# johanna-rock/quantization_analysis

Hardware: AMD Instinct MI355X
Metric: 32x32 tiles/s for mixed-tile-greedy (bf16->BFP{8,4,2}); achieved HBM GB/s vs peak (higher is better)
Workload: dtype f32/f64

## Files before the change

### include/mtq.h

```cpp
#ifndef MTQ_H
#define MTQ_H

#include <stddef.h>
#include <stdint.h>

#ifdef __cplusplus
extern "C" {
#endif

#define MTQ_VERSION 143

typedef enum {
    MTQ_OK = 0,
    MTQ_ERR_INVALID = -1,
    MTQ_ERR_HIP = -2,
    MTQ_ERR_NO_DEVICE = -3,
    MTQ_ERR_UNSUPPORTED = -4
} mtq_status;

enum { MTQ_DTYPE_BF16 = 0, MTQ_DTYPE_F32 = 1 };

enum { MTQ_FMT_BF16 = 0, MTQ_FMT_BFP8 = 1, MTQ_FMT_BFP4 = 2, MTQ_FMT_BFP2 = 3, MTQ_FMT_FP0 = 4, MTQ_FMT_MXFP4 = 5, MTQ_FMT_NVFP4 = 6 };
#define MTQ_NUM_TILE_FORMATS 4
#define MTQ_MASK_ALL 0xFu
// ... 130 lines not shown

int mtq_tile_scores_device(const double *stats, int64_t tiles, uint32_t fmt_mask, int metric, double *scores, void *stream);

int mtq_threshold_assign_device(const double *stats, int64_t tiles, uint32_t fmt_mask, const int *formats, int n_formats,
                                int metric, double threshold, double band, int8_t *map, uint8_t *knife, void *stream);


size_t mtq_columns_scratch_doubles(void);
int mtq_column_sums_device(const double *stats, int64_t tiles, uint32_t fmt_mask, const int8_t *map, double *scratch, void *stream);
int mtq_column_sums_device_batched(const double *stats, int64_t count, int64_t tiles, uint32_t fmt_mask, const int8_t *maps,
                                   double *scratch, void *stream);

#define MTQ_SCAN_DEVICE_MAX_TILES (1 << 22)
size_t mtq_greedy_scan_scratch_bytes(int64_t count, int64_t tiles);
int mtq_greedy_scan_device(const double *stats, int64_t count, int64_t tiles, uint32_t fmt_mask, const int *formats, int n_formats,
                           int metric, double threshold, double elem_count, const uint64_t *seeds, int8_t *maps, int32_t *status,
                           int32_t *counts, void *scratch, size_t scratch_bytes, void *stream);

size_t mtq_scan_carry_bytes(int64_t count);
int mtq_greedy_scan_device_ex(const double *stats, int64_t count, int64_t tiles, uint32_t fmt_mask, const int *formats, int n_formats,
                              int metric, double threshold, double elem_count, const uint64_t *seeds, int8_t *maps, int32_t *status,
                              int32_t *counts, void *scratch, size_t scratch_bytes, const void *orders, int phase, uint32_t *listed,
                              uint32_t *n_listed, void *carry, void *stream);
size_t mtq_scan_orders_bytes(int64_t tiles);
int mtq_scan_orders_device(uint64_t seed, int64_t tiles, int n_orders, void *orders, size_t orders_bytes, void *stream);

int mtq_knife_tiles_device(const void *x, int in_dtype, int64_t count, int64_t stride_elems, int64_t rows, int64_t cols, int64_t ld,
                           const int8_t *near, const int *formats, int n_formats, int64_t cap, int64_t *list, float *tiles_out, void *stream);

int mtq_knife_tiles_transposed(const void *x, int in_dtype, int64_t count, int64_t stride_elems, int64_t rows, int64_t cols, int64_t ld,
                               const int8_t *near, const int *formats, int n_formats, int64_t cap, int64_t *list, float *tiles_out, void *stream);

int mtq_threshold_enqueue(const void *x, int in_dtype, int64_t count, int64_t stride_elems, int64_t rows, int64_t cols, int64_t ld,
                          uint32_t k1_mask, uint32_t dec_mask, const int *formats, int n_formats, int metric, double threshold, double band,
                          double *stats, int8_t *both_dev, int8_t *both_host, int64_t cap, int64_t *list_dev, float *knife_dev,
                          int64_t *list_host, double *scratch, double *sums_host, void *stream, void *side_stream);
int mtq_threshold_enqueue_transposed(const void *x, int in_dtype, int64_t count, int64_t stride_elems, int64_t rows, int64_t cols, int64_t ld,
                                     uint32_t k1_mask, uint32_t dec_mask, const int *formats, int n_formats, int metric, double threshold, double band,
                                     double *stats, int8_t *both_dev, int8_t *both_host, int64_t cap, int64_t *list_dev, float *knife_dev,
                                     int64_t *list_host, double *scratch, double *sums_host, void *stream, void *side_stream);
int mtq_threshold_columns(const double *stats, int64_t count, int64_t tiles, uint32_t dec_mask, const int8_t *maps_dev, double *scratch,
                          double *sums_host, void *stream);

#define MTQ_RAGGED_MAX 24
typedef struct MtqMatrix { const void *x; int64_t rows, cols, ld; } MtqMatrix;
int mtq_tile_stats_ragged(const MtqMatrix *mats, int n, int in_dtype, uint32_t fmt_mask, double *stats, void *stream);
// ... 25 lines not shown
```

### quantization_analysis_amd/csrc/mtq_decide.hip

```cpp
#include <hip/hip_runtime.h>
#include <stdint.h>

#include "../../include/mtq.h"
#include "mtq_decide.hpp"
#include "mtq_error.hpp"

namespace mtq {

struct SlotTable { int slot[MTQ_NUM_TILE_FORMATS]; };

__global__ __launch_bounds__(256) void tile_scores_dev(const double *__restrict__ stats, int64_t tiles, int rec, SlotTable st, int metric,
                                                       double *__restrict__ scores)
{
    const int64_t t = (int64_t)blockIdx.x * 256 + threadIdx.x;
    if (t >= tiles) return;
    const double *r = stats + t * rec;
    int64_t row = 0;
#pragma unroll
    for (int f = 0; f < MTQ_NUM_TILE_FORMATS; ++f) {
        if (!slot_ok(st.slot[f])) continue;
        scores[row * tiles + t] = tile_score(r, st.slot[f], metric);
        ++row;
    }
}

__global__ __launch_bounds__(256) void threshold_assign_dev(const double *__restrict__ stats, int64_t tiles, int rec, ThresholdPlan plan,
                                                            int metric, double thr32, double band, int8_t *__restrict__ map,
                                                            uint8_t *__restrict__ knife)
{
    const int64_t t = (int64_t)blockIdx.x * 256 + threadIdx.x;
    if (t >= tiles) return;
    unsigned near;
    map[t] = (int8_t)threshold_decide(stats + t * rec, plan, metric, thr32, band, near);
    knife[t] = (uint8_t)near;
}

constexpr int kColBlocks = 256, kColVals = 11, kColMax = 6;

constexpr int kColSegs = 24;
struct ColSegs { uint32_t n; uint32_t first[kColSegs + 1]; };

__global__ __launch_bounds__(256) void columns_partial_dev(const double *__restrict__ stats, int64_t tiles, int rec, SlotTable st,
                                                           const int8_t *__restrict__ map, double *__restrict__ partial, int64_t scratch_stride,
                                                           const ColSegs seg)
{
    __shared__ double red[kColVals][256];
    int64_t stride_blocks = gridDim.x;
    if (seg.n) {
        const int64_t first = seg.first[blockIdx.y];
        tiles = (int64_t)seg.first[blockIdx.y + 1] - first;
        stride_blocks = (tiles + 255) / 256 < kColBlocks ? (tiles + 255) / 256 : kColBlocks;
        if ((int64_t)blockIdx.x >= stride_blocks) return;
        stats += first * rec;
        map += first;
    } else {
        stats += (int64_t)blockIdx.y * tiles * rec;
        map += (int64_t)blockIdx.y * tiles;
    }
    partial += (int64_t)blockIdx.y * scratch_stride;
    double v[kColVals] = {0, 0, 0, 0, 0, 0, 0, 0, 0, 0, 0};
// ... 233 lines not shown
```

### quantization_analysis_amd/csrc/mtq_decide.hpp

```cpp
#pragma once
#include <stdint.h>

#include "../../include/mtq.h"

#if defined(__HIP__)
#define MTQ_HD __host__ __device__
#else
#define MTQ_HD
#endif

namespace mtq {

MTQ_HD inline int popcount4(uint32_t m) { return __builtin_popcount(m & MTQ_MASK_ALL); }

constexpr int kVirtualSlot = -2;

MTQ_HD inline int slot_of(uint32_t mask, int f)
{
    if (f < 0 || f >= MTQ_NUM_TILE_FORMATS) return -1;
    if (f == 0 && (mask & MTQ_MASK_BF16_IDENTITY) && !(mask & 1u)) return kVirtualSlot;
    if (!(mask & (1u << f))) return -1;
    return __builtin_popcount(mask & ((1u << f) - 1u));
}
MTQ_HD inline bool slot_ok(int slot) { return slot >= 0 || slot == kVirtualSlot; }

struct Sums5 { double y, y2, xy, ab, mx; };
MTQ_HD inline Sums5 load5(const double *r, int slot)
{
    if (slot >= 0) { const double *b = r + 2 + 5 * slot; return {b[0], b[1], b[2], b[3], b[4]}; }
    const double z = __builtin_fabs(r[0]) * 0.0;
    return {r[0], r[1], r[1], z, z};
}

MTQ_HD inline double nanmax(double m, double d) { return (d > m || d != d) ? d : m; }

MTQ_HD inline bool is_good(double v, int metric, double thr) { return metric == MTQ_METRIC_PCC ? v >= thr : v <= thr; }

MTQ_HD inline double pcc_from_moments(double n, double sx, double sx2, double sy, double sy2, double sxy, double sab)
{
    if (n == 0.0) return 1.0;
    const double mean_x = sx / n;
    const double mean_y = sy / n;
    double am2 = sx2 - n * mean_x * mean_x;
    double bm2 = sy2 - n * mean_y * mean_y;
    if (am2 < 0.0) am2 = 0.0;
    if (bm2 < 0.0) bm2 = 0.0;
    const double denom = __builtin_sqrt(am2 * bm2);
    if (denom == 0.0) return sab == 0.0 ? 1.0 : 0.0;
    return (sxy - n * mean_x * mean_y) / denom;
}

MTQ_HD inline double tile_score(const double *r, int slot, int metric)
{
    const Sums5 b = load5(r, slot);
    if (metric == MTQ_METRIC_MAE) return b.ab / 1024.0;
    if (metric == MTQ_METRIC_ATOL) return b.mx;
    return pcc_from_moments(1024.0, r[0], r[1], b.y, b.y2, b.xy, b.ab);
// ... 52 lines not shown
```

### quantization_analysis_amd/csrc/mtq_scan.hip

```cpp
#include <hip/hip_runtime.h>
#include <stdint.h>

#include <atomic>
#include <type_traits>
#include <stdlib.h>
#include <mutex>

#include "../../include/mtq.h"
#include "mtq_decide.hpp"
#include "mtq_error.hpp"

namespace mtq {
namespace {

constexpr int kScanMaxTilesLds = 32768;
constexpr int kTagSlots = 16384;
constexpr int kJump = 34;

} }
__device__ unsigned long long g_scan_ticks[16];
namespace mtq { namespace {

struct U128 { uint64_t lo, hi; };
__host__ __device__ inline U128 mul128(U128 a, U128 b)
// ... 232 lines not shown
struct ScanArgs {
    const double *stats;
    int64_t tiles;
    int rec;
    int n_formats;
    int fmt[MTQ_NUM_TILE_FORMATS];
    int oy[MTQ_NUM_TILE_FORMATS], oy2[MTQ_NUM_TILE_FORMATS], oxy[MTQ_NUM_TILE_FORMATS];
    int oab[MTQ_NUM_TILE_FORMATS];
    int omx[MTQ_NUM_TILE_FORMATS];
    int metric;
    double thr, n;
    const uint64_t *seeds;
    int8_t *maps;
    int32_t *status;
    int32_t *counts;
    uint32_t *order_g;
    double *delta;
    double *delta2;
    const U128 *jump_a, *jump_g;
    const unsigned char *orders;
    int phase;
    uint32_t *listed, *n_listed;
    Carry *carry;
};

constexpr int kNoOffset = 0xFF;
__device__ inline double rec_at(const double *rt, uint32_t off) { return off == (uint32_t)kNoOffset ? 0.0 : rt[off]; }

template <int kN>
__device__ inline void prefix_chain(const double *lds_d, double *lds_p, int lane, double s)
{
    double v[16], w[16];
#pragma unroll
    for (int u = 0; u < 16; ++u) v[u] = lds_d[u * 4 + lane];
#pragma unroll
    for (int i0 = 0; i0 < kN; i0 += 16) {
        if (i0 + 16 < kN) {
#pragma unroll
            for (int u = 0; u < 16; ++u) w[u] = lds_d[(i0 + 16 + u) * 4 + lane];
        }
#pragma unroll
        for (int u = 0; u < 16; ++u) { s = s + v[u]; lds_p[(i0 + u) * 4 + lane] = s; }
#pragma unroll
        for (int u = 0; u < 16; ++u) v[u] = w[u];
    }
}
// ... 25 lines not shown
    special = denom == 0.0;
    const double val = (sxy - n * mean_x * mean_y) / denom;
    return val >= thr;
}

#ifdef MTQ_SCAN_PROFILE
#define MTQ_SCAN_STAMP(slot) do { const unsigned long long now_ = clock64(); if (b == 0 && lane == 0 && (slot) < 16) g_scan_ticks[slot] = now_ - tick_s; tick_s = now_; } while (0)
#else
#define MTQ_SCAN_STAMP(slot) do { } while (0)
#endif

template <typename F>
__device__ __forceinline__ void sift_map(const int8_t *map, int T, int lane, F &&f)
{
    for (int t00 = 0; t00 < T; t00 += 64 * 8) {
        uint8_t b[8];
#pragma unroll
        for (int u = 0; u < 8; ++u) b[u] = (uint8_t)ld_l2(map + min(t00 + 64 * u + lane, T - 1));
#pragma unroll
        for (int u = 0; u < 8; ++u) b[u] = t00 + 64 * u + lane < T ? b[u] : (uint8_t)0x80u;
#pragma unroll
        for (int u = 0; u < 8; ++u)
            if (t00 + 64 * u < T) f(t00 + 64 * u, b[u]);
    }
}

struct Offsets3 { uint32_t y, y2, xy; };

template <bool kMae, typename TileAt, typename PrevOf>
__device__ inline void gather_deltas(const double *st, int rec, Offsets3 po, int f, int nc, double *delta, int lane, TileAt tile_at, PrevOf prev_of)
{
    const uint32_t oy_f = (po.y >> (8 * f)) & 0xFFu, oy2_f = (po.y2 >> (8 * f)) & 0xFFu, oxy_f = (po.xy >> (8 * f)) & 0xFFu;
    uint32_t nt[4];
#pragma unroll
    for (int u = 0; u < 4; ++u) {
        const int k = 64 * u + lane;
        nt[u] = k < nc ? tile_at((uint32_t)k) : 0u;
    }
    for (int k0 = 0; k0 < nc; k0 += 256) {
        uint32_t tt[4];
        int pv[4];
#pragma unroll
        for (int u = 0; u < 4; ++u) tt[u] = nt[u];
#pragma unroll
        for (int u = 0; u < 4; ++u) {
            const int k = k0 + 256 + 64 * u + lane;
// ... 418 lines not shown
        }
        if (lane == 0) {
            Carry &c = a.carry[b];
            c.Sy = Sy; c.Sy2 = Sy2; c.Sxy = Sxy; c.sum_x = sum_x; c.sum_x2 = sum_x2;
            c.state = r.state; c.inc = inc; c.has32 = r.has32 ? 1u : 0u; c.u32 = r.u32;
            c.status = status; c.done = (done || nc == 0) ? 1 : 0;
        }
        return;
    }

    int per_fmt[MTQ_NUM_TILE_FORMATS] = {0, 0, 0, 0};
    sift_map(map, T, lane, [&](int t0, uint8_t raw) {
        const int t = t0 + lane;
        int code = -1;
        if (t < T) { code = (int)(raw & 0x7Fu); map[t] = (int8_t)code; }
#pragma unroll
        for (int c = 0; c < MTQ_NUM_TILE_FORMATS; ++c) per_fmt[c] += __builtin_popcountll(__ballot(code == c));
    });
    if (lane == 0) {
        a.status[b] = status;
        if (a.counts)
            for (int c = 0; c < MTQ_NUM_TILE_FORMATS; ++c) a.counts[b * MTQ_NUM_TILE_FORMATS + c] = per_fmt[c];
    }
}

__global__ __launch_bounds__(256) void greedy_atol(ScanArgs a)
{
    __shared__ int s_bad, s_nan, s_cnt[MTQ_NUM_TILE_FORMATS];
    const int b = blockIdx.x;
    const int64_t T = a.tiles;
    const double *st = a.stats + (int64_t)b * T * a.rec;
    int8_t *map = a.maps + (int64_t)b * T;
    if (threadIdx.x == 0) { s_bad = 0; s_nan = 0; }
    if (threadIdx.x < MTQ_NUM_TILE_FORMATS) s_cnt[threadIdx.x] = 0;
    __syncthreads();
    const int base = a.fmt[0];
    bool bad = false, nan = false;
    for (int64_t t = threadIdx.x; t < T; t += 256) {
        const double *rt = st + t * a.rec;
        bad |= !(rec_at(rt, (uint32_t)a.omx[base]) <= a.thr);
        for (int p = 0; p < a.n_formats; ++p) { const double v = rec_at(rt, (uint32_t)a.omx[a.fmt[p]]); nan |= v != v; }
    }
    if (bad) s_bad = 1;
    if (nan) s_nan = 1;
    __syncthreads();
    const bool all_base = s_bad != 0;
// ... 177 lines not shown
{
    if (!orders) return fail(MTQ_ERR_INVALID, "null argument");
    if (seed == 0) return fail(MTQ_ERR_INVALID, "seed 0 means 'draw a random seed' in the reference; pass a non-zero seed");
    if (tiles <= 0 || tiles > MTQ_SCAN_DEVICE_MAX_TILES) return fail(MTQ_ERR_INVALID, "tiles out of range");
    if (n_orders < 1 || n_orders > 2) return fail(MTQ_ERR_INVALID, "n_orders must be 1 or 2");
    if (orders_bytes < mtq_scan_orders_bytes(tiles)) return fail(MTQ_ERR_INVALID, "orders is smaller than mtq_scan_orders_bytes()");
    if (int rc = require_device()) return rc;
    int dev = 0;
    if (hipGetDevice(&dev) != hipSuccess) return fail(MTQ_ERR_HIP, "hipGetDevice failed");
    const U128 *jt = jump_tables(dev);
    if (!jt) return fail(MTQ_ERR_HIP, "could not upload the jump-ahead tables");
    OrdersArgs a{seed, tiles, n_orders, static_cast<unsigned char *>(orders), jt, jt + kJump};
    hipStream_t st = static_cast<hipStream_t>(stream);
    if (hipMemsetAsync(orders, 0, sizeof(OrdersHdr), st) != hipSuccess) return fail(MTQ_ERR_HIP, "hipMemsetAsync failed");
    size_t lds = kTagSlots;
    if (tiles <= kScanMaxTilesLds) {
        lds += 2 * (size_t)((tiles + 7) & ~(int64_t)7);
        if (int rc = raise_lds(dev, 1, reinterpret_cast<const void *>(scan_orders), 2 * kScanMaxTilesLds + kTagSlots)) return rc;
    }
    hipLaunchKernelGGL(scan_orders, dim3((unsigned)n_orders), dim3(64), lds, st, a);
    return check_launch("mtq_scan_orders_device");
}

extern "C" int mtq_greedy_scan_device_ex(const double *stats, int64_t count, int64_t tiles, uint32_t fmt_mask, const int *formats, int n_formats,
                                         int metric, double threshold, double elem_count, const uint64_t *seeds, int8_t *maps, int32_t *status,
                                         int32_t *counts, void *scratch, size_t scratch_bytes, const void *orders, int phase, uint32_t *listed,
                                         uint32_t *n_listed, void *carry, void *stream)
{
    if (!stats || !formats || !seeds || !maps || !status || !scratch) return fail(MTQ_ERR_INVALID, "null argument");
    if (count <= 0 || count > (1 << 20) || tiles <= 0) return fail(MTQ_ERR_INVALID, "count and tiles must be positive");
    if (tiles > MTQ_SCAN_DEVICE_MAX_TILES) return fail(MTQ_ERR_UNSUPPORTED, "more tiles than the device scan takes: use the host scan");
    if (metric != MTQ_METRIC_PCC && metric != MTQ_METRIC_MAE && metric != MTQ_METRIC_ATOL) return fail(MTQ_ERR_INVALID, "unknown metric");
    if (n_formats <= 0 || n_formats > MTQ_NUM_TILE_FORMATS) return fail(MTQ_ERR_INVALID, "n_formats must be 1..4");
    if (fmt_mask & MTQ_MASK_SLIM) return fail(MTQ_ERR_INVALID, "the device scan reads full records");
    if (!(elem_count > 0.0)) return fail(MTQ_ERR_INVALID, "elem_count must be positive");
    if (scratch_bytes < mtq_greedy_scan_scratch_bytes(count, tiles)) return fail(MTQ_ERR_INVALID, "scratch is smaller than mtq_greedy_scan_scratch_bytes()");
    if (phase < 0 || phase > 2) return fail(MTQ_ERR_INVALID, "phase must be 0, 1 or 2");
    if (phase != 0) {
        if (metric == MTQ_METRIC_ATOL) return fail(MTQ_ERR_UNSUPPORTED, "the atol walk has no phases");
        if (n_formats < 2) return fail(MTQ_ERR_INVALID, "a split search needs at least two formats");
        if (!carry || (phase == 1 && (!listed || !n_listed))) return fail(MTQ_ERR_INVALID, "a split search needs carry (and listed, n_listed in phase 1)");
        if (count * tiles >= ((int64_t)1 << 32)) return fail(MTQ_ERR_INVALID, "too many tiles for the list of a split search");
    }
    ScanArgs a{};
    a.stats = stats;
    a.tiles = tiles;
    a.rec = 2 + 5 * popcount4(fmt_mask);
    a.n_formats = n_formats;
    for (int f = 0; f < MTQ_NUM_TILE_FORMATS; ++f) {
        const int s = slot_of(fmt_mask, f);
        a.oy[f] = s >= 0 ? 2 + 5 * s : 0;
        a.oy2[f] = s >= 0 ? 3 + 5 * s : 1;
        a.oxy[f] = s >= 0 ? 4 + 5 * s : 1;
        a.oab[f] = s >= 0 ? 5 + 5 * s : kNoOffset;
        a.omx[f] = s >= 0 ? 6 + 5 * s : kNoOffset;
    }
    a.metric = metric;
    for (int i = 0; i < n_formats; ++i) {
        if (!slot_ok(slot_of(fmt_mask, formats[i]))) return fail(MTQ_ERR_INVALID, "a format is not available under fmt_mask");
        for (int j = 0; j < i; ++j) if (formats[j] == formats[i]) return fail(MTQ_ERR_UNSUPPORTED, "the device scan needs distinct formats: use the host scan");
        a.fmt[i] = formats[i];
    }
    a.thr = threshold;
    a.n = elem_count;
    a.seeds = seeds;
    a.maps = maps;
    a.status = status;
    a.counts = counts;
    a.orders = static_cast<const unsigned char *>(orders);
    a.phase = phase;
    a.listed = listed;
    a.n_listed = n_listed;
    a.carry = static_cast<Carry *>(carry);
    if (int rc = require_device()) return rc;
    int dev = 0;
    if (hipGetDevice(&dev) != hipSuccess) return fail(MTQ_ERR_HIP, "hipGetDevice failed");
    const U128 *jt = jump_tables(dev);
    if (!jt) return fail(MTQ_ERR_HIP, "could not upload the jump-ahead tables");
    a.jump_a = jt;
    a.jump_g = jt + kJump;
    a.delta = static_cast<double *>(scratch);
    a.delta2 = a.delta + (size_t)count * (size_t)tiles * 4;
    a.order_g = reinterpret_cast<uint32_t *>(static_cast<unsigned char *>(scratch) + (size_t)count * (size_t)tiles * 8 * sizeof(double));
    hipStream_t st = static_cast<hipStream_t>(stream);
    if (metric == MTQ_METRIC_ATOL) {
        hipLaunchKernelGGL(greedy_atol, dim3((unsigned)count), dim3(256), 0, st, a);
        return check_launch("mtq_greedy_scan_device");
    }
    const unsigned threads = (orders && phase != 2) ? 128u : 64u;
    static int shared_lds = -1;
    if (shared_lds < 0) { const char *e = getenv("MTQ_SCAN_SHARED_LDS"); shared_lds = e ? atoi(e) : 0; }
    if (tiles <= kScanMaxTilesLds && !(threads == 128u && !shared_lds)) {
        const size_t lds = 2 * (size_t)((tiles + 7) & ~(int64_t)7) + kFixedLds;
        if (int rc = raise_lds(dev, 0, reinterpret_cast<const void *>(greedy_scan_pcc_lds), 2 * kScanMaxTilesLds + (int)kFixedLds)) return rc;
        hipLaunchKernelGGL(greedy_scan_pcc_lds, dim3((unsigned)count), dim3(threads), lds, st, a);
    } else {
        hipLaunchKernelGGL(greedy_scan_pcc_global, dim3((unsigned)count), dim3(threads), kFixedLds, st, a);
    }
    return check_launch("mtq_greedy_scan_device");
}

extern "C" int mtq_greedy_scan_device(const double *stats, int64_t count, int64_t tiles, uint32_t fmt_mask, const int *formats, int n_formats,
                                      int metric, double threshold, double elem_count, const uint64_t *seeds, int8_t *maps, int32_t *status,
                                      int32_t *counts, void *scratch, size_t scratch_bytes, void *stream)
{
    return mtq_greedy_scan_device_ex(stats, count, tiles, fmt_mask, formats, n_formats, metric, threshold, elem_count, seeds, maps, status, counts,
                                     scratch, scratch_bytes, nullptr, 0, nullptr, nullptr, nullptr, stream);
}
```

### quantization_analysis_amd/hip_backend.py

```python
from __future__ import annotations

import ctypes
import functools
import os
from pathlib import Path

import numpy as np

_PKG = Path(__file__).resolve().parent
LIB_PATH = Path(os.environ["MTQ_LIB"]).resolve() if os.environ.get("MTQ_LIB") else _PKG / "libmtq_hip.so"

MIXED_TILE_FORMATS = ["bf16", "bfp8", "bfp4", "bfp2"]
FMT_CODE = {"bf16": 0, "bfp8": 1, "bfp4": 2, "bfp2": 3, "fp0": 4}
PROXY_FORMATS = ["mxfp4", "nvfp4"]
QUANTIZE_CODE = {**FMT_CODE, "mxfp4": 5, "nvfp4": 6}
METRIC_CODE = {"pcc": 0, "mae": 1, "atol": 2}
DTYPE_BF16, DTYPE_F32 = 0, 1
TILE = 32

MTQ_VERSION = 143

SIGNATURES = {
    "mtq_version": ("i", "", False),
    "mtq_last_error": ("s", "", False),
# ... 18 lines not shown
    "mtq_greedy_value": ("i", "pp", False),
    "mtq_greedy_destroy": ("v", "p", False),
    "mtq_tile_scores": ("i", "pluip", False),
    "mtq_threshold_assign": ("i", "plupiiddppplp", False),
    "mtq_columns_from_stats": ("i", "plupdp", False),
    "mtq_columns_from_sums": ("i", "pdp", False),
    "mtq_tile_scores_device": ("i", "pluipp", False),
    "mtq_threshold_assign_device": ("i", "plupiiddppp", False),
    "mtq_columns_scratch_doubles": ("z", "", False),
    "mtq_column_sums_device": ("i", "pluppp", False),
    "mtq_column_sums_device_batched": ("i", "plluppp", False),
    "mtq_rng_create": ("i", "pq", False),
    "mtq_rng_permutation": ("i", "plp", False),
    "mtq_rng_integers": ("i", "pllp", False),
    "mtq_rng_destroy": ("v", "p", False),
    "mtq_greedy_run": ("i", "plupiiddqppp", False),
    "mtq_greedy_run_batch": ("i", "pllupiiddppppi", False),
    "mtq_selftest_slot_ring": ("i", "", False),
    "mtq_device_copy_2d": ("i", "pzpzzzp", False),
    "mtq_knife_tiles_device": ("i", "pilllllppilppp", False),
    "mtq_greedy_scan_scratch_bytes": ("z", "ll", False),
    "mtq_greedy_scan_device": ("i", "pllupiiddpppppzp", False),
    "mtq_greedy_scan_device_ex": ("i", "pllupiiddpppppzpipppp", False),
    "mtq_scan_carry_bytes": ("z", "l", False),
    "mtq_scan_orders_bytes": ("z", "l", False),
    "mtq_scan_orders_device": ("i", "qlipzp", False),
    "mtq_debug_scan_ticks": ("i", "p", False),
    "mtq_threshold_enqueue": ("i", "pillllluupiiddppplppppppp", False),
    "mtq_threshold_columns": ("i", "pllupppp", False),
    "mtq_tile_stats_ragged": ("i", "piiupp", False),
    "mtq_knife_tiles_ragged": ("i", "piippilppp", False),
    "mtq_column_sums_device_ragged": ("i", "ppiuppp", False),
    "mtq_threshold_enqueue_ragged": ("i", "piiuupiiddppplppppppp", False),
    "mtq_threshold_columns_ragged": ("i", "ppiupppp", False),
    "mtq_tile_stats_transposed": ("i", "pilllllupp", True),
    "mtq_quantize_transposed": ("i", "pillliplp", True),
    "mtq_apply_assignment_transposed": ("i", "pilllllpplp", True),
    "mtq_knife_tiles_transposed": ("i", "pilllllppilppp", True),
    "mtq_threshold_enqueue_transposed": ("i", "pillllluupiiddppplppppppp", True),
    "mtq_output_error_scratch_doubles": ("z", "ll", True),
    "mtq_output_error": ("i", "plllpillpuppilppzp", True),
    "mtq_fp4_proxy_scratch_doubles": ("z", "lll", True),
    "mtq_fp4_proxy_sums": ("i", "pillllluppzp", True),
    "mtq_output_error_qx": ("i", "plllpillpuppilppzppl", True),
    "mtq_quantize_rows_bf16": ("i", "pllliplp", True),
    "mtq_gram_blocks_scratch_doubles": ("z", "ll", True),
# ... 816 lines not shown
    if scratch is None:
        scratch = torch.empty((need,), dtype=torch.uint8, device=stats_dev.device)
    elif scratch.numel() < need:
        raise ValueError(f"scratch holds {scratch.numel()} bytes, mtq_greedy_scan_scratch_bytes() asks for {need}")
    check(lib().mtq_greedy_scan_device(stats_dev.data_ptr(), count, T, mask, fm, len(formats), METRIC_CODE[metric], float(threshold),
                                       float(elem_count), seeds_dev.data_ptr(), maps.data_ptr(), status.data_ptr(),
                                       counts_out.data_ptr() if counts_out is not None else None, scratch.data_ptr(), int(scratch.numel()), _stream_ptr()))
    return maps, status


def scan_orders_device(seed: int, tiles: int, n_orders: int = 2, out=None):
    torch = _torch()
    require_gpu()
    need = int(lib().mtq_scan_orders_bytes(int(tiles)))
    if out is None:
        out = torch.empty((need,), dtype=torch.uint8, device="cuda")
    elif out.numel() < need:
        raise ValueError("orders buffer is smaller than mtq_scan_orders_bytes()")
    check(lib().mtq_scan_orders_device(int(seed), int(tiles), int(n_orders), out.data_ptr(), int(out.numel()), _stream_ptr()))
    return out


def greedy_scan_device_ex(stats_dev, mask: int, formats, metric: str, threshold: float, elem_count: float, seeds_dev, maps_out, status_out,
                          scratch, counts_out=None, orders=None, phase: int = 0, listed=None, n_listed=None, carry=None) -> None:
    count, T = int(stats_dev.shape[0]), int(stats_dev.shape[1])
    need = greedy_scan_scratch_bytes(count, T)
    if scratch.numel() < need:
        raise ValueError("scratch is smaller than mtq_greedy_scan_scratch_bytes()")
    fm = _format_codes(formats)
    check(lib().mtq_greedy_scan_device_ex(stats_dev.data_ptr(), count, T, mask, fm, len(formats), METRIC_CODE[metric], float(threshold), float(elem_count),
                                          seeds_dev.data_ptr(), maps_out.data_ptr(), status_out.data_ptr(),
                                          counts_out.data_ptr() if counts_out is not None else None, scratch.data_ptr(), int(scratch.numel()),
                                          orders.data_ptr() if orders is not None else None, int(phase),
                                          listed.data_ptr() if listed is not None else None, n_listed.data_ptr() if n_listed is not None else None,
                                          carry.data_ptr() if carry is not None else None, _stream_ptr()))


def tile_stats_listed(x3d, layout_mask: int, full_mask: int, err_mask: int, listed, n_listed, stats, scratch=None) -> None:
    require_gpu()
    code, count, stride, rows, cols, ld = _contiguous_batch(x3d)
    check(lib().mtq_tile_stats_listed(x3d.data_ptr(), code, count, stride, rows, cols, ld, layout_mask, full_mask, err_mask,
                                      listed.data_ptr(), n_listed.data_ptr(), int(listed.numel()),
                                      scratch.data_ptr() if scratch is not None else None, stats.data_ptr(), _stream_ptr()))


def greedy_run_batch(stats: np.ndarray, mask: int, formats, metric: str, threshold: float, elem_count: float, seeds, n_threads: int):
    stats = np.ascontiguousarray(stats, dtype=np.float64)
    count, T = stats.shape[0], stats.shape[1]
    fm = _format_codes(formats)
    sd = np.ascontiguousarray(seeds, dtype=np.uint64)
    maps = np.empty((count, T), dtype=np.int8)
    counts = np.empty((count, 4), dtype=np.int64)
# ... 179 lines not shown
```

### quantization_analysis_amd/pipeline_greedy.py

```python
from __future__ import annotations

import concurrent.futures as cf
import contextlib
import os
import time
from dataclasses import dataclass, field

import numpy as np

from . import hip_backend as hb
from .compression_algorithms.tile_utils import MIXED_TILE_FORMATS, mixed_tile_total_bytes
from .settings import settings
from .pipeline_common import KernelTiming, TensorResult, _scan_chunk, _sleep_until, _when_landed, columns_from_sums_batch, gated_pcc


class GreedyPipeline:

    SLOTS = None

    def __init__(self, tile_formats=None, metric: str = "pcc", threshold: float = 0.999, seed: int = 123,
                 chunk: int = 8, workers: int = 8, pure_formats=(), scan: str = "auto", scan_streams: int | None = None, layout: str = "rows"):
        import torch

        hb.require_gpu()
# ... 10 lines not shown
        self.chunk = int(chunk)
        self.workers = int(workers)
        self.pool = cf.ThreadPoolExecutor(max_workers=settings().chunk_tasks)
        self.stream = torch.cuda.Stream()
        self.copy_stream = torch.cuda.Stream()
        self.col_stream = torch.cuda.Stream()
        self.timing = KernelTiming()
        self.SLOTS = type(self).SLOTS or settings().pipe_slots
        if scan not in ("auto", "host", "device"):
            raise ValueError("scan must be 'auto', 'host' or 'device'")
        can = hb.device_scan_supported(self.tile_formats, self.metric, 1)
        if scan == "device" and not can:
            raise ValueError("the device scan needs distinct formats")
        self.device_scan = can and scan != "host" and settings().device_scan
        self.device_scan_max_tiles = settings().device_scan_max_tiles or hb.SCAN_DEVICE_MAX_TILES
        self.host_chunk_tiles = None
        n_scan = settings().scan_streams if settings().scan_streams is not None else (3 if scan_streams is None else scan_streams)
        self.scan_streams = [torch.cuda.Stream(priority=settings().scan_priority)
                             for _ in range(max(1, n_scan))]
        self._scan_rr = 0
        self.shared_orders = settings().shared_orders
        self.lazy = (settings().lazy and self.metric == "pcc" and len(self.tile_formats) >= 3 and self.tile_formats[0] == "bf16"
                     and len(set(self.tile_formats)) == len(self.tile_formats) and not self.pure_formats and not self.transposed)
        self.listed_tiles = 0
        self.lazy_max_listed = settings().lazy_max_listed
        self.lazy_off = {}
        self.host_fallbacks = 0
        self.host_seconds = {"enqueue": 0.0, "wait": 0.0, "wrap": 0.0}
        self._devbufs = {}
        self._orders_cache = {}
        self._orders_retired = []
        self._bufs = {}
        self._colbufs = {}
        self._unresolved = []
        self._open = []
        self._next_slot = 0

    def _layout(self, x3d):
        torch = self.torch
        identity = x3d.dtype == torch.bfloat16 and (self.mask & 1) and (self.mask & 0xE) and settings().identity_records
        k1_mask = self.mask & 0xE if identity else self.mask
        host_mask = k1_mask | hb.MASK_BF16_IDENTITY if identity else self.mask
        slim = self.metric == "pcc" and settings().slim_records
        return k1_mask, host_mask | (hb.MASK_SLIM if slim else 0), slim

    def _grid(self, rows: int, cols: int) -> tuple[int, int]:
# ... 91 lines not shown
                if slim:
                    hb.pack_slim_records(dev[first:first + n], k1_mask, out=stage[first:first + n])
                    ready = torch.cuda.Event()
                    ready.record(self.stream)
                self.copy_stream.wait_event(ready)
                with torch.cuda.stream(self.copy_stream):
                    host[first:first + n].copy_(stage[first:first + n], non_blocking=True)
                    done = torch.cuda.Event(blocking=True)
                    done.record(self.copy_stream)
                pending.append((done, first, n))
        enq = {"host_np": host_np, "host_mask": host_mask, "tiles_hw": (th, tw), "numel": rows * cols if numel is None else int(numel),
               "seeds": seeds, "x": x3d, "dev": dev, "k1_mask": k1_mask, "slim": slim}
        futures = []
        for done, first, n in pending:
            futures.append((first, n, self.pool.submit(_when_landed, done, _scan_chunk, *self._scan_args(enq, first, n, host_np[first:first + n], host_mask))))
        enq["futures"] = futures
        self._open.append(enq)
        if trace:
            print(f"[pipe] enqueue (host route) {count} x {tiles} tiles in chunks of {chunk}: buffers {1e3 * (t_buf - t_enq):.2f}, launches {1e3 * (time.perf_counter() - t_buf):.2f} ms", flush=True)
        return enq

    def _use_device_scan(self, tiles: int) -> bool:
        return self.device_scan and tiles <= self.device_scan_max_tiles and hb.device_scan_supported(self.tile_formats, self.metric, tiles)

    def _host_chunk(self, count: int, tiles: int) -> int:
        if self.host_chunk_tiles is None:
            return self.chunk
        return min(max(1, self.host_chunk_tiles // tiles), count)

    def _device_buffers(self, slot: int, count: int, tiles: int, rec: int, device) -> dict:
        torch = self.torch
        b = self._devbufs.get(slot)
        if b is None or b["device"] != str(device):
            b = {"device": str(device), "flat": {}, "key": None}
            self._devbufs[slot] = b
        key = (count, tiles, rec)
        if b["key"] == key:
            return b
        n_scratch = hb.columns_scratch_doubles()
        P = 1 + len(self.pure_formats)
        nf = len(MIXED_TILE_FORMATS)

        def flat(name, numel, dtype, pinned=False):
            t = b["flat"].get(name)
            if t is None or t.numel() < numel:
                t = torch.zeros((int(numel * 1.25) + 16,), dtype=dtype, pin_memory=True) if pinned else \
# ... 91 lines not shown
                    hb.tile_stats_partial(x3d[first:first + n], k1_mask, full_now, prev_bit, out=b["dev"][first:first + n])
                else:
                    self._k1(x3d[first:first + n], k1_mask, out=b["dev"][first:first + n])
                e1.record(self.stream)
            self.timing.events.append((e0, e1, n * tiles))
            if trace:
                marks.append(("k1", time.perf_counter()))
            scan_stream.wait_event(e1)
            if trace:
                if getattr(self, "_trace_ref", None) is None:
                    self._trace_ref = e0
                    self._trace_t0 = time.perf_counter()
            with torch.cuda.stream(scan_stream):
                b["seeds_dev"][first:first + n].copy_(b["seeds_host"][first:first + n], non_blocking=True)
                recs = b["dev"][first:first + n]
                maps = b["maps_dev"][first:first + n]
                if k1_id is not None:
                    hb.tile_stats_partial_end(x3d[first:first + n], k1_mask, recs, b["mark"][ci:ci + 1], k1_id)
                if shared and orders_ready is not None:
                    scan_stream.wait_event(orders_ready)
                args = (recs, dec_mask, self.tile_formats, self.metric, self.threshold, float(n_el), b["seeds_dev"][first:first + n], maps,
                        b["status_dev"][first:first + n], b["scratch"][first * per:(first + n) * per])
                orders = orders_buf if shared else None
                if lazy:
                    xs = x3d[first:first + n]
                    listed, nl = b["listed"][first * tiles:(first + n) * tiles], b["n_listed"][ci:ci + 1]
                    carry = b["carry"][first * per_carry:(first + n) * per_carry]
                    nl.zero_()
                    hb.greedy_scan_device_ex(*args, counts_out=b["counts_dev"][first:first + n], orders=orders, phase=1, listed=listed, n_listed=nl, carry=carry)
                    hb.tile_stats_listed(xs, k1_mask, last_bit, prev_bit, listed, nl, recs, scratch=b["lscr"][first * tiles + ci:(first + n) * tiles + ci + 1])
                    hb.greedy_scan_device_ex(*args, counts_out=b["counts_dev"][first:first + n], phase=2, carry=carry)
                else:
                    hb.greedy_scan_device_ex(*args, counts_out=b["counts_dev"][first:first + n], orders=orders)
                hb.column_sums_device_batched(recs, n, tiles, dec_mask, maps, b["sums_dev"][0, first:first + n], scan_stream)
                for k, pm in enumerate(b["pure_maps"]):
                    hb.column_sums_device_batched(recs, n, tiles, dec_mask, pm[first:first + n], b["sums_dev"][1 + k, first:first + n], scan_stream)
                scanned = torch.cuda.Event(enable_timing=trace)
                scanned.record(scan_stream)
            if trace:
                marks.append(("scan+sums", time.perf_counter()))
            with torch.cuda.stream(scan_stream):
                hb.device_copy(b["maps_host"][first:first + n], maps)
                hb.device_copy(b["status_host"][first:first + n], b["status_dev"][first:first + n])
                hb.device_copy(b["counts_host"][first:first + n], b["counts_dev"][first:first + n])
                if lazy:
                    hb.device_copy(b["n_listed_host"][ci:ci + 1], b["n_listed"][ci:ci + 1])
                for q in range(b["sums_dev"].shape[0]):
                    hb.device_copy(b["sums_host"][q, first:first + n], b["sums_dev"][q, first:first + n, :7])
                done = torch.cuda.Event(blocking=True, enable_timing=trace)
                done.record(scan_stream)
            pending.append((done, first, n))
            if trace:
                self._trace_rows = getattr(self, "_trace_rows", []) + [(count, tiles, e0, e1, scanned, done, time.perf_counter())]
        enq = {"device": True, "buf": b, "pending": pending, "tiles_hw": (th, tw), "numel": n_el, "x": x3d, "dec_mask": dec_mask,
               "seeds": sh.copy(), "lazy": lazy, "k1_mask": k1_mask}
        self._open.append(enq)
        self.host_seconds["enqueue"] += time.perf_counter() - t_enq
# ... 326 lines not shown
```

### quantization_analysis_amd/settings.py

```python
from __future__ import annotations

import os
from dataclasses import dataclass


def _flag(name: str, default: bool) -> bool:
    v = os.environ.get(name)
    return default if v is None else v != "0"


def _int(name: str, default: int | None) -> int | None:
    v = os.environ.get(name)
    return default if v is None else int(v)


@dataclass(frozen=True)
class Settings:
    pipe_slots: int
    scan_streams: int | None
    scan_priority: int
    chunk_tasks: int
    scan_workers: int | None
    device_scan: bool
    device_scan_max_tiles: int | None
    shared_orders: bool
    lazy: bool
    lazy_max_listed: float
    identity_records: bool
    slim_records: bool
    k1_two_launch: bool
    knife_cap: int
    threshold_ragged: bool
    sweep_threads: int | None
    wq_max_slots: int
    wq_device_scan_max_tiles: int
    pipe_trace: bool
    numa_bind: bool


_CACHED: Settings | None = None


def settings(refresh: bool = False) -> Settings:
    global _CACHED
    if _CACHED is None or refresh:
        _CACHED = Settings(
            pipe_slots=_int("MTQ_PIPE_SLOTS", 4), scan_streams=_int("MTQ_SCAN_STREAMS", None), scan_priority=_int("MTQ_SCAN_PRIORITY", -1),
            chunk_tasks=_int("MTQ_CHUNK_TASKS", 8), scan_workers=_int("MTQ_SCAN_WORKERS", None), device_scan=_flag("MTQ_DEVICE_SCAN", True),
            device_scan_max_tiles=_int("MTQ_DEVICE_SCAN_MAX_TILES", None), shared_orders=_flag("MTQ_SHARED_ORDERS", True), lazy=_flag("MTQ_LAZY", True),
            lazy_max_listed=float(os.environ.get("MTQ_LAZY_MAX_LISTED", "0.35")), identity_records=_flag("MTQ_IDENTITY_RECORDS", True),
            slim_records=_flag("MTQ_SLIM_RECORDS", True), k1_two_launch=_flag("MTQ_K1_TWO_LAUNCH", True), knife_cap=_int("MTQ_KNIFE_CAP", 128), threshold_ragged=_flag("MTQ_THRESHOLD_RAGGED", True),
            sweep_threads=_int("MTQ_SWEEP_THREADS", None), wq_max_slots=_int("MTQ_WQ_MAX_SLOTS", 8),
            wq_device_scan_max_tiles=_int("MTQ_WQ_DEVICE_SCAN_MAX_TILES", 1 << 22), pipe_trace=os.environ.get("MTQ_PIPE_TRACE") == "1",
            numa_bind=_flag("MTQ_NUMA_BIND", True))
    return _CACHED
```

Measured before the change: 1.274 billion.

## Fuse column sums into the greedy scan kernel tail for small tile counts

Adds a column-sum walk that runs at the end of the device greedy scan. It reuses the just-written map to accumulate per-format statistics with a software-pipelined ring of record and map loads, plus wave-level shuffle reductions. When fusion is chosen, the separate column_sums_device_batched launch for the greedy map is skipped. Fusion is the default only for non-lazy scans with at most 16384 tiles and the pcc or mae metric. This removes a kernel launch and a re-read of the map and stats, but adds serial work and register pressure to the scan wave.

Result: slower. 1.258 billion (-1.3%).

```diff
diff --git a/include/mtq.h b/include/mtq.h
--- a/include/mtq.h
+++ b/include/mtq.h
@@ -176,6 +176,10 @@
                               int metric, double threshold, double elem_count, const uint64_t *seeds, int8_t *maps, int32_t *status,
                               int32_t *counts, void *scratch, size_t scratch_bytes, const void *orders, int phase, uint32_t *listed,
                               uint32_t *n_listed, void *carry, void *stream);
+int mtq_greedy_scan_device_sums(const double *stats, int64_t count, int64_t tiles, uint32_t fmt_mask, const int *formats, int n_formats,
+                                int metric, double threshold, double elem_count, const uint64_t *seeds, int8_t *maps, int32_t *status,
+                                int32_t *counts, void *scratch, size_t scratch_bytes, const void *orders, int phase, uint32_t *listed,
+                                uint32_t *n_listed, void *carry, double *sums_scratch, void *stream);
 size_t mtq_scan_orders_bytes(int64_t tiles);
 int mtq_scan_orders_device(uint64_t seed, int64_t tiles, int n_orders, void *orders, size_t orders_bytes, void *stream);
 
diff --git a/quantization_analysis_amd/csrc/mtq_decide.hip b/quantization_analysis_amd/csrc/mtq_decide.hip
--- a/quantization_analysis_amd/csrc/mtq_decide.hip
+++ b/quantization_analysis_amd/csrc/mtq_decide.hip
@@ -34,8 +34,6 @@
     map[t] = (int8_t)threshold_decide(stats + t * rec, plan, metric, thr32, band, near);
     knife[t] = (uint8_t)near;
 }
-
-constexpr int kColBlocks = 256, kColVals = 11, kColMax = 6;
 
 constexpr int kColSegs = 24;
 struct ColSegs { uint32_t n; uint32_t first[kColSegs + 1]; };
diff --git a/quantization_analysis_amd/csrc/mtq_decide.hpp b/quantization_analysis_amd/csrc/mtq_decide.hpp
--- a/quantization_analysis_amd/csrc/mtq_decide.hpp
+++ b/quantization_analysis_amd/csrc/mtq_decide.hpp
@@ -32,7 +32,24 @@
     return {r[0], r[1], r[1], z, z};
 }
 
+struct Raw7 { double x, x2, v[5]; };
+template <bool kWide>
+MTQ_HD inline Raw7 load7(const double *r, int slot)
+{
+    if (!kWide) return {r[0], r[1], {0.0, 0.0, 0.0, 0.0, 0.0}};
+    const double *b = slot >= 0 ? r + 2 + 5 * slot : r;
+    return {r[0], r[1], {b[0], b[1], b[2], b[3], b[4]}};
+}
+MTQ_HD inline Sums5 sums5(const Raw7 &q, int slot)
+{
+    if (slot >= 0) return {q.v[0], q.v[1], q.v[2], q.v[3], q.v[4]};
+    const double z = __builtin_fabs(q.x) * 0.0;
+    return {q.x, q.x2, q.x2, z, z};
+}
+
 MTQ_HD inline double nanmax(double m, double d) { return (d > m || d != d) ? d : m; }
+
+constexpr int kColBlocks = 256, kColVals = 11, kColMax = 6;
 
 MTQ_HD inline bool is_good(double v, int metric, double thr) { return metric == MTQ_METRIC_PCC ? v >= thr : v <= thr; }
 
diff --git a/quantization_analysis_amd/csrc/mtq_scan.hip b/quantization_analysis_amd/csrc/mtq_scan.hip
--- a/quantization_analysis_amd/csrc/mtq_scan.hip
+++ b/quantization_analysis_amd/csrc/mtq_scan.hip
@@ -278,6 +278,8 @@
     int phase;
     uint32_t *listed, *n_listed;
     Carry *carry;
+    double *sums;
+    uint32_t slot_pk;
 };
 
 constexpr int kNoOffset = 0xFF;
@@ -349,6 +351,130 @@
 #pragma unroll
         for (int u = 0; u < 8; ++u)
             if (t00 + 64 * u < T) f(t00 + 64 * u, b[u]);
+    }
+}
+
+struct ColIter { int b, h, k; };
+struct ColChunk { Raw7 q[2]; int meta[2]; };
+
+__device__ __forceinline__ void col_next(ColIter &it, int stride, int T)
+{
+    ++it.k;
+    if (it.b * 256 + it.k * stride >= T) { it.k = 0; if (++it.h == 2) { it.h = 0; ++it.b; } }
+}
+
+__device__ __forceinline__ double col_tree(double g, int lane, bool is_max)
+{
+#pragma unroll
+    for (int s = 32; s > 0; s >>= 1) {
+        const double o = shfl_f64(g, (lane + s) & 63);
+        g = is_max ? nanmax(g, o) : g + o;
+    }
+    return g;
+}
+
+template <bool kWide, bool kSingle, int kColRing>
+__device__ __forceinline__ void column_sums_walk(const double *st, int rec, const int8_t *map, int T, uint32_t slot_pk, double *out, int lane)
+{
+    const int B = min((T + 255) / 256, kColBlocks), stride = B * 256;
+    double *part = out + kColVals;
+    ColIter ci{0, 0, 0}, ri = ci, mi = ci;
+    ColChunk ring[kColRing];
+    constexpr int kColMapAhead = kColRing;
+    uint8_t mb[kColMapAhead][2];
+    auto tile_of = [&](const ColIter &it, int e) { return it.b * 256 + 64 * (it.h + 2 * e) + lane + it.k * stride; };
+    auto ask_map = [&](uint8_t (&m)[2], const ColIter &it) {
+#pragma unroll
+        for (int e = 0; e < 2; ++e) m[e] = (uint8_t)ld_l2(map + min(tile_of(it, e), T - 1));
+    };
+    auto ask_records = [&](ColChunk &c, const uint8_t (&m)[2], const ColIter &it) {
+#pragma unroll
+        for (int e = 0; e < 2; ++e) {
+            const int t = tile_of(it, e);
+            const int f = m[e] & 0x7F;
+            const int slot = f < MTQ_NUM_TILE_FORMATS ? (int)((slot_pk >> (8 * (f & 3))) & 0xFFu) - 2 : -1;
+            c.q[e] = load7<kWide>(st + (int64_t)min(t, T - 1) * rec, slot);
+            c.meta[e] = t < T ? (slot_ok(slot) ? (f | (slot < 0 ? 8 : 0)) : 4) : -1;
+        }
+    };
+    double acc[2][7], half0[7];
+    int cntb[MTQ_NUM_TILE_FORMATS] = {0, 0, 0, 0}, tot[MTQ_NUM_TILE_FORMATS] = {0, 0, 0, 0};
+#pragma unroll
+    for (int j = 0; j < 7; ++j) acc[0][j] = acc[1][j] = half0[j] = 0.0;
+    auto add_chunk = [&](const ColChunk &c, const ColIter &it) {
+        if (kSingle || it.k == 0) {
+#pragma unroll
+            for (int j = 0; j < 7; ++j) acc[0][j] = acc[1][j] = 0.0;
+        }
+#pragma unroll
+        for (int e = 0; e < 2; ++e) {
+            const int meta = c.meta[e];
+            const bool live = meta >= 0 && meta != 4;
+            const Sums5 s = sums5(c.q[e], (meta & 8) ? kVirtualSlot : 0);
+            const double val[6] = {c.q[e].x, c.q[e].x2, s.y, s.y2, s.xy, s.ab};
+#pragma unroll
+            for (int j = 0; j < 6; ++j) acc[e][j] = live ? acc[e][j] + val[j] : acc[e][j];
+            if (meta == 4) acc[e][0] = __builtin_nan("");
+            acc[e][kColMax] = live ? nanmax(acc[e][kColMax], s.mx) : acc[e][kColMax];
+#pragma unroll
+            for (int f = 0; f < MTQ_NUM_TILE_FORMATS; ++f) cntb[f] += __builtin_popcountll(__ballot(live && (meta & 7) == f));
+        }
+        if (!kSingle && it.b * 256 + (it.k + 1) * stride < T) return;
+        double g[7];
+#pragma unroll
+        for (int j = 0; j < 7; ++j) g[j] = j == kColMax ? nanmax(acc[0][j], acc[1][j]) : acc[0][j] + acc[1][j];
+        if (it.h == 0) {
+#pragma unroll
+            for (int j = 0; j < 7; ++j) half0[j] = g[j];
+            return;
+        }
+#pragma unroll
+        for (int j = 0; j < 7; ++j) g[j] = col_tree(j == kColMax ? nanmax(half0[j], g[j]) : half0[j] + g[j], lane, j == kColMax);
+        if (lane == 0) {
+#pragma unroll
+            for (int j = 0; j < 7; ++j) part[it.b * kColVals + j] = g[j];
+#pragma unroll
+            for (int f = 0; f < MTQ_NUM_TILE_FORMATS; ++f) part[it.b * kColVals + 7 + f] = (double)cntb[f];
+        }
+#pragma unroll
+        for (int f = 0; f < MTQ_NUM_TILE_FORMATS; ++f) { tot[f] += cntb[f]; cntb[f] = 0; }
+    };
+#pragma unroll
+    for (int u = 0; u < kColMapAhead; ++u) { ask_map(mb[u], mi); col_next(mi, stride, T); }
+#pragma unroll
+    for (int u = 0; u < kColRing; ++u) {
+        ask_records(ring[u], mb[u], ri); col_next(ri, stride, T);
+        ask_map(mb[u], mi); col_next(mi, stride, T);
+    }
+    while (ci.b < B) {
+#pragma unroll
+        for (int u = 0; u < kColRing; ++u) {
+            if (ci.b < B) add_chunk(ring[u], ci);
+            col_next(ci, stride, T);
+            ask_records(ring[u], mb[u], ri); col_next(ri, stride, T);
+            ask_map(mb[u], mi); col_next(mi, stride, T);
+        }
+    }
+    mem_wait();
+    double p[4][7];
+#pragma unroll
+    for (int q = 0; q < 4; ++q)
+#pragma unroll
+        for (int j = 0; j < 7; ++j) p[q][j] = ld_l2(part + min(64 * q + lane, B - 1) * kColVals + j);
+#pragma unroll
+    for (int q = 0; q < 4; ++q)
+#pragma unroll
+        for (int j = 0; j < 7; ++j) p[q][j] = 64 * q + lane < B ? p[q][j] : 0.0;
+#pragma unroll
+    for (int j = 0; j < 7; ++j) {
+        const bool mx = j == kColMax;
+        const double a02 = mx ? nanmax(p[0][j], p[2][j]) : p[0][j] + p[2][j], a13 = mx ? nanmax(p[1][j], p[3][j]) : p[1][j] + p[3][j];
+        const double g = col_tree(mx ? nanmax(a02, a13) : a02 + a13, lane, mx);
+        if (lane == 0) out[j] = g;
+    }
+    if (lane == 0) {
+#pragma unroll
+        for (int f = 0; f < MTQ_NUM_TILE_FORMATS; ++f) out[7 + f] = (double)tot[f];
     }
 }
 
@@ -813,6 +939,12 @@
         if (a.counts)
             for (int c = 0; c < MTQ_NUM_TILE_FORMATS; ++c) a.counts[b * MTQ_NUM_TILE_FORMATS + c] = per_fmt[c];
     }
+    if (a.sums) {
+        double *out = a.sums + (int64_t)b * (kColVals * (kColBlocks + 1));
+        if (rec >= 7 && T <= 256 * kColBlocks) column_sums_walk<true, true, 4>(st, rec, map, T, a.slot_pk, out, lane);
+        else if (rec >= 7) column_sums_walk<true, false, 3>(st, rec, map, T, a.slot_pk, out, lane);
+        else column_sums_walk<false, false, 3>(st, rec, map, T, a.slot_pk, out, lane);
+    }
 }
 
 __global__ __launch_bounds__(256) void greedy_atol(ScanArgs a)
@@ -1036,10 +1168,10 @@
     return check_launch("mtq_scan_orders_device");
 }
 
-extern "C" int mtq_greedy_scan_device_ex(const double *stats, int64_t count, int64_t tiles, uint32_t fmt_mask, const int *formats, int n_formats,
-                                         int metric, double threshold, double elem_count, const uint64_t *seeds, int8_t *maps, int32_t *status,
-                                         int32_t *counts, void *scratch, size_t scratch_bytes, const void *orders, int phase, uint32_t *listed,
-                                         uint32_t *n_listed, void *carry, void *stream)
+extern "C" int mtq_greedy_scan_device_sums(const double *stats, int64_t count, int64_t tiles, uint32_t fmt_mask, const int *formats, int n_formats,
+                                           int metric, double threshold, double elem_count, const uint64_t *seeds, int8_t *maps, int32_t *status,
+                                           int32_t *counts, void *scratch, size_t scratch_bytes, const void *orders, int phase, uint32_t *listed,
+                                           uint32_t *n_listed, void *carry, double *sums_scratch, void *stream)
 {
     if (!stats || !formats || !seeds || !maps || !status || !scratch) return fail(MTQ_ERR_INVALID, "null argument");
     if (count <= 0 || count > (1 << 20) || tiles <= 0) return fail(MTQ_ERR_INVALID, "count and tiles must be positive");
@@ -1056,6 +1188,10 @@
         if (!carry || (phase == 1 && (!listed || !n_listed))) return fail(MTQ_ERR_INVALID, "a split search needs carry (and listed, n_listed in phase 1)");
         if (count * tiles >= ((int64_t)1 << 32)) return fail(MTQ_ERR_INVALID, "too many tiles for the list of a split search");
     }
+    if (sums_scratch) {
+        if (phase == 1) return fail(MTQ_ERR_INVALID, "phase 1 leaves no finished map to sum: pass sums_scratch to phase 2");
+        if (metric == MTQ_METRIC_ATOL) return fail(MTQ_ERR_UNSUPPORTED, "the atol walk does not sum columns: use mtq_column_sums_device_batched");
+    }
     ScanArgs a{};
     a.stats = stats;
     a.tiles = tiles;
@@ -1086,6 +1222,8 @@
     a.listed = listed;
     a.n_listed = n_listed;
     a.carry = static_cast<Carry *>(carry);
+    a.sums = sums_scratch;
+    for (int f = 0; f < MTQ_NUM_TILE_FORMATS; ++f) a.slot_pk |= (uint32_t)(slot_of(fmt_mask, f) + 2) << (8 * f);
     if (int rc = require_device()) return rc;
     int dev = 0;
     if (hipGetDevice(&dev) != hipSuccess) return fail(MTQ_ERR_HIP, "hipGetDevice failed");
@@ -1114,6 +1252,15 @@
     return check_launch("mtq_greedy_scan_device");
 }
 
+extern "C" int mtq_greedy_scan_device_ex(const double *stats, int64_t count, int64_t tiles, uint32_t fmt_mask, const int *formats, int n_formats,
+                                         int metric, double threshold, double elem_count, const uint64_t *seeds, int8_t *maps, int32_t *status,
+                                         int32_t *counts, void *scratch, size_t scratch_bytes, const void *orders, int phase, uint32_t *listed,
+                                         uint32_t *n_listed, void *carry, void *stream)
+{
+    return mtq_greedy_scan_device_sums(stats, count, tiles, fmt_mask, formats, n_formats, metric, threshold, elem_count, seeds, maps, status, counts,
+                                       scratch, scratch_bytes, orders, phase, listed, n_listed, carry, nullptr, stream);
+}
+
 extern "C" int mtq_greedy_scan_device(const double *stats, int64_t count, int64_t tiles, uint32_t fmt_mask, const int *formats, int n_formats,
                                       int metric, double threshold, double elem_count, const uint64_t *seeds, int8_t *maps, int32_t *status,
                                       int32_t *counts, void *scratch, size_t scratch_bytes, void *stream)
diff --git a/quantization_analysis_amd/hip_backend.py b/quantization_analysis_amd/hip_backend.py
--- a/quantization_analysis_amd/hip_backend.py
+++ b/quantization_analysis_amd/hip_backend.py
@@ -64,6 +64,7 @@
     "mtq_greedy_scan_scratch_bytes": ("z", "ll", False),
     "mtq_greedy_scan_device": ("i", "pllupiiddpppppzp", False),
     "mtq_greedy_scan_device_ex": ("i", "pllupiiddpppppzpipppp", False),
+    "mtq_greedy_scan_device_sums": ("i", "pllupiiddpppppzpippppp", True),
     "mtq_scan_carry_bytes": ("z", "l", False),
     "mtq_scan_orders_bytes": ("z", "l", False),
     "mtq_scan_orders_device": ("i", "qlipzp", False),
@@ -926,12 +927,25 @@
 
 
 def greedy_scan_device_ex(stats_dev, mask: int, formats, metric: str, threshold: float, elem_count: float, seeds_dev, maps_out, status_out,
-                          scratch, counts_out=None, orders=None, phase: int = 0, listed=None, n_listed=None, carry=None) -> None:
+                          scratch, counts_out=None, orders=None, phase: int = 0, listed=None, n_listed=None, carry=None, sums_out=None) -> None:
     count, T = int(stats_dev.shape[0]), int(stats_dev.shape[1])
     need = greedy_scan_scratch_bytes(count, T)
     if scratch.numel() < need:
         raise ValueError("scratch is smaller than mtq_greedy_scan_scratch_bytes()")
     fm = _format_codes(formats)
+    if sums_out is not None:
+        torch = _torch()
+        n_scratch = columns_scratch_doubles()
+        if (sums_out.dtype != torch.float64 or not sums_out.is_cuda or tuple(sums_out.shape) != (count, n_scratch) or sums_out.stride(1) != 1
+                or (count > 1 and sums_out.stride(0) != n_scratch)):
+            raise ValueError("sums_out must be a float64 device tensor [count, columns_scratch_doubles()] with contiguous rows")
+        check(_entry("mtq_greedy_scan_device_sums")(
+            stats_dev.data_ptr(), count, T, mask, fm, len(formats), METRIC_CODE[metric], float(threshold), float(elem_count),
+            seeds_dev.data_ptr(), maps_out.data_ptr(), status_out.data_ptr(), counts_out.data_ptr() if counts_out is not None else None,
+            scratch.data_ptr(), int(scratch.numel()), orders.data_ptr() if orders is not None else None, int(phase),
+            listed.data_ptr() if listed is not None else None, n_listed.data_ptr() if n_listed is not None else None,
+            carry.data_ptr() if carry is not None else None, sums_out.data_ptr(), _stream_ptr()))
+        return
     check(lib().mtq_greedy_scan_device_ex(stats_dev.data_ptr(), count, T, mask, fm, len(formats), METRIC_CODE[metric], float(threshold), float(elem_count),
                                           seeds_dev.data_ptr(), maps_out.data_ptr(), status_out.data_ptr(),
                                           counts_out.data_ptr() if counts_out is not None else None, scratch.data_ptr(), int(scratch.numel()),
diff --git a/quantization_analysis_amd/pipeline_greedy.py b/quantization_analysis_amd/pipeline_greedy.py
--- a/quantization_analysis_amd/pipeline_greedy.py
+++ b/quantization_analysis_amd/pipeline_greedy.py
@@ -56,6 +56,7 @@
         self.shared_orders = settings().shared_orders
         self.lazy = (settings().lazy and self.metric == "pcc" and len(self.tile_formats) >= 3 and self.tile_formats[0] == "bf16"
                      and len(set(self.tile_formats)) == len(self.tile_formats) and not self.pure_formats and not self.transposed)
+        self.fused_columns = settings().fused_columns
         self.listed_tiles = 0
         self.lazy_max_listed = settings().lazy_max_listed
         self.lazy_off = {}
@@ -193,6 +194,15 @@
 
     def _use_device_scan(self, tiles: int) -> bool:
         return self.device_scan and tiles <= self.device_scan_max_tiles and hb.device_scan_supported(self.tile_formats, self.metric, tiles)
+
+    FUSED_COLUMNS_MAX_TILES = 16384
+
+    def _fuse_columns(self, tiles: int, lazy: bool) -> bool:
+        if self.metric not in ("pcc", "mae"):
+            return False
+        if self.fused_columns is not None:
+            return self.fused_columns
+        return not lazy and tiles <= self.FUSED_COLUMNS_MAX_TILES
 
     def _host_chunk(self, count: int, tiles: int) -> int:
         if self.host_chunk_tiles is None:
@@ -330,6 +340,7 @@
                 args = (recs, dec_mask, self.tile_formats, self.metric, self.threshold, float(n_el), b["seeds_dev"][first:first + n], maps,
                         b["status_dev"][first:first + n], b["scratch"][first * per:(first + n) * per])
                 orders = orders_buf if shared else None
+                sums_out = b["sums_dev"][0, first:first + n] if self._fuse_columns(tiles, lazy) else None
                 if lazy:
                     xs = x3d[first:first + n]
                     listed, nl = b["listed"][first * tiles:(first + n) * tiles], b["n_listed"][ci:ci + 1]
@@ -337,10 +348,11 @@
                     nl.zero_()
                     hb.greedy_scan_device_ex(*args, counts_out=b["counts_dev"][first:first + n], orders=orders, phase=1, listed=listed, n_listed=nl, carry=carry)
                     hb.tile_stats_listed(xs, k1_mask, last_bit, prev_bit, listed, nl, recs, scratch=b["lscr"][first * tiles + ci:(first + n) * tiles + ci + 1])
-                    hb.greedy_scan_device_ex(*args, counts_out=b["counts_dev"][first:first + n], phase=2, carry=carry)
+                    hb.greedy_scan_device_ex(*args, counts_out=b["counts_dev"][first:first + n], phase=2, carry=carry, sums_out=sums_out)
                 else:
-                    hb.greedy_scan_device_ex(*args, counts_out=b["counts_dev"][first:first + n], orders=orders)
-                hb.column_sums_device_batched(recs, n, tiles, dec_mask, maps, b["sums_dev"][0, first:first + n], scan_stream)
+                    hb.greedy_scan_device_ex(*args, counts_out=b["counts_dev"][first:first + n], orders=orders, sums_out=sums_out)
+                if sums_out is None:
+                    hb.column_sums_device_batched(recs, n, tiles, dec_mask, maps, b["sums_dev"][0, first:first + n], scan_stream)
                 for k, pm in enumerate(b["pure_maps"]):
                     hb.column_sums_device_batched(recs, n, tiles, dec_mask, pm[first:first + n], b["sums_dev"][1 + k, first:first + n], scan_stream)
                 scanned = torch.cuda.Event(enable_timing=trace)
diff --git a/quantization_analysis_amd/settings.py b/quantization_analysis_amd/settings.py
--- a/quantization_analysis_amd/settings.py
+++ b/quantization_analysis_amd/settings.py
@@ -25,6 +25,7 @@
     device_scan_max_tiles: int | None
     shared_orders: bool
     lazy: bool
+    fused_columns: bool | None
     lazy_max_listed: float
     identity_records: bool
     slim_records: bool
@@ -48,6 +49,7 @@
             pipe_slots=_int("MTQ_PIPE_SLOTS", 4), scan_streams=_int("MTQ_SCAN_STREAMS", None), scan_priority=_int("MTQ_SCAN_PRIORITY", -1),
             chunk_tasks=_int("MTQ_CHUNK_TASKS", 8), scan_workers=_int("MTQ_SCAN_WORKERS", None), device_scan=_flag("MTQ_DEVICE_SCAN", True),
             device_scan_max_tiles=_int("MTQ_DEVICE_SCAN_MAX_TILES", None), shared_orders=_flag("MTQ_SHARED_ORDERS", True), lazy=_flag("MTQ_LAZY", True),
+            fused_columns=None if os.environ.get("MTQ_FUSED_COLUMNS") is None else _flag("MTQ_FUSED_COLUMNS", True),
             lazy_max_listed=float(os.environ.get("MTQ_LAZY_MAX_LISTED", "0.35")), identity_records=_flag("MTQ_IDENTITY_RECORDS", True),
             slim_records=_flag("MTQ_SLIM_RECORDS", True), k1_two_launch=_flag("MTQ_K1_TWO_LAUNCH", True), knife_cap=_int("MTQ_KNIFE_CAP", 128), threshold_ragged=_flag("MTQ_THRESHOLD_RAGGED", True),
             sweep_threads=_int("MTQ_SWEEP_THREADS", None), wq_max_slots=_int("MTQ_WQ_MAX_SLOTS", 8),
```
